# bioinfo-ut/GenomeTester4

Hardware: AMD Instinct MI355X
Metric: k-mers merged/sec, 2-list k=25 intersection (glistcompare -i), lists resident in HBM (higher is better)
Workload: dtype u64 keys + u32 counts

## Files before the change

### genometester4_amd/capi.py

```python
from __future__ import annotations

import ctypes as C
import os

import numpy as np

from .listio import RECORD_DTYPE

PKG_DIR = os.path.dirname(os.path.abspath(__file__))
LIB_PATH = os.environ.get("GT4HIP_LIB") or os.path.join(PKG_DIR, "libgt4hip.so")

OK = 0
EINVAL, ENODEVICE, ENOMEM, ERULE, EHIP, EWORDLEN, EINTERNAL = 1, 2, 3, 4, 5, 6, 7
EFORMAT = 11
MAKER_FORWARD_ONLY, MAKER_TEXT_ON_DEVICE = 1, 2
MAKER_ERR_START, MAKER_ERR_PLUS, MAKER_ERR_AT, MAKER_ERR_PLUS_EOF = 1, 2, 3, 4
OP_UNION, OP_INTRSEC, OP_DIFF1, OP_DIFF2 = 1, 2, 4, 8
RULE_DEFAULT, RULE_ADD, RULE_SUBTRACT, RULE_MIN, RULE_MAX, RULE_FIRST, RULE_SECOND, RULE_NUMBER = range(8)


class CompareParams(C.Structure):
    _fields_ = [("ops", C.c_uint32), ("rule", C.c_int32), ("cutoff", C.c_uint32), ("subtract", C.c_int32),
                ("count_override", C.c_uint32), ("count_only", C.c_int32)]

# ... 61 lines not shown


class MultiResult(C.Structure):
    _fields_ = [("n_words", C.c_uint64), ("total_count", C.c_uint64), ("out", C.c_void_p), ("device_ms", C.c_double),
                ("records_read", C.c_uint64), ("records_written", C.c_uint64)]


class CountTable(C.Structure):
    _fields_ = [("n_keys", C.c_uint64), ("n_lists", C.c_uint32), ("device_keys", C.c_void_p),
                ("device_counts", C.c_void_p), ("owner", C.c_void_p * 2), ("ragged", C.c_void_p)]


SYMBOLS = [
    "gt4hip_create", "gt4hip_destroy", "gt4hip_last_error", "gt4hip_strerror", "gt4hip_device_count",
    "gt4hip_device_info", "gt4hip_list_upload", "gt4hip_list_upload_index", "gt4hip_list_wrap", "gt4hip_list_alloc", "gt4hip_list_slice",
    "gt4hip_list_download", "gt4hip_list_download_range", "gt4hip_list_free", "gt4hip_list_n_words",
    "gt4hip_list_word_length", "gt4hip_list_device_ptr", "gt4hip_list_set_n_words", "gt4hip_list_sum_counts",
    "gt4hip_list_is_sorted", "gt4hip_list_lower_bound", "gt4hip_list_get_word", "gt4hip_compare",
    "gt4hip_union_multi", "gt4hip_intersect_multi", "gt4hip_union_table", "gt4hip_probe_table", "gt4hip_probe_table_ex", "gt4hip_table_compact", "gt4hip_table_download",
    "gt4hip_table_free", "gt4hip_generate", "gt4hip_generate_ex", "gt4hip_synchronize", "gt4hip_set_option",
    "gt4hip_get_counter", "gt4hip_device_memory", "gt4hip_list_upload_fd", "gt4hip_list_load_fd", "gt4hip_list_load",
    "gt4hip_list_write_fd", "gt4hip_lists_write_fd", "gt4hip_shard_first_key", "gt4hip_shard_cuts", "gt4hip_comm_unique_id", "gt4hip_comm_create", "gt4hip_comm_destroy", "gt4hip_comm_allgather_totals", "gt4hip_comm_allgather_u64", "gt4hip_context_device", "gt4hip_trim",
    "gt4hip_comm_rank", "gt4hip_comm_size", "gt4hip_comm_last_error", "gt4hip_comm_gatherv", "gt4hip_sort_words", "gt4hip_words_to_list",
    "gt4hip_device_words_to_list", "gt4hip_compare_mismatch", "gt4hip_mismatch_stats_get",
    "gt4hip_query_index_create", "gt4hip_query_index_free", "gt4hip_query_index_last_ms", "gt4hip_query_variants",
    "gt4hip_query_variant_mask", "gt4hip_query_lookup", "gt4hip_query_lookup_all", "gt4hip_list_count_stats",
    "gt4hip_list_count_split", "gt4hip_list_count_histogram", "gt4hip_list_gc",
    "gt4hip_location_index_create", "gt4hip_location_index_free", "gt4hip_location_index_list", "gt4hip_location_index_n_locations",
    "gt4hip_query_lookup_locations", "gt4hip_query_index_gather_ms",
    "gt4hip_text_to_words", "gt4hip_words_free", "gt4hip_words_download", "gt4hip_text_to_list",
    "gt4hip_sort_pairs", "gt4hip_pairs_to_index", "gt4hip_index_free",
    "gt4hip_list_subset", "gt4hip_subset_state_at",
    "gt4hip_text_to_locations", "gt4hip_locations_free", "gt4hip_pack_locations", "gt4hip_pairs_reserve", "gt4hip_pairs_release",
]

_lib = None


class Gt4HipError(RuntimeError):
    def __init__(self, code, msg):
        super().__init__("gt4hip error %d: %s" % (code, msg))
        self.code = code


def lib():
    global _lib
    if _lib is None:
        if not os.path.exists(LIB_PATH):
            raise ImportError("%s is missing: build it with `make -C genometester4_amd/csrc` "
                              "(there is no CPU fallback)" % LIB_PATH)
        L = C.CDLL(LIB_PATH)
        vp, u64, u32, i32 = C.c_void_p, C.c_uint64, C.c_uint32, C.c_int32
        sig = {
            "gt4hip_create": (C.c_int, [C.c_int, C.POINTER(vp)]),
            "gt4hip_destroy": (None, [vp]),
            "gt4hip_last_error": (C.c_char_p, [vp]),
            "gt4hip_strerror": (C.c_char_p, [C.c_int]),
            "gt4hip_device_count": (C.c_int, []),
            "gt4hip_device_info": (C.c_char_p, [vp]),
            "gt4hip_list_upload": (C.c_int, [vp, vp, u64, u32, C.POINTER(vp)]),
            "gt4hip_list_upload_index": (C.c_int, [vp, vp, u64, u64, u32, C.POINTER(vp)]),
            "gt4hip_list_wrap": (C.c_int, [vp, vp, u64, u32, C.POINTER(vp)]),
            "gt4hip_list_alloc": (C.c_int, [vp, u64, u32, C.POINTER(vp)]),
            "gt4hip_list_slice": (C.c_int, [vp, vp, u64, u64, C.POINTER(vp)]),
            "gt4hip_list_download": (C.c_int, [vp, vp, vp]),
            "gt4hip_list_download_range": (C.c_int, [vp, vp, u64, u64, vp]),
# ... 45 lines not shown
            "gt4hip_query_index_create": (C.c_int, [vp, vp, C.POINTER(vp)]),
            "gt4hip_query_index_free": (None, [vp]),
            "gt4hip_query_index_last_ms": (C.c_double, [vp]),
            "gt4hip_query_variants": (C.c_int, [u32, C.POINTER(QueryParams), C.POINTER(u64)]),
            "gt4hip_query_variant_mask": (C.c_int, [u32, C.POINTER(QueryParams), u64, C.POINTER(u64)]),
            "gt4hip_query_lookup": (C.c_int, [vp, vp, vp, u64, C.POINTER(QueryParams), vp, vp]),
            "gt4hip_query_lookup_all": (C.c_int, [vp, vp, vp, u64, C.POINTER(QueryParams), vp, u64, C.POINTER(u64)]),
            "gt4hip_location_index_create": (C.c_int, [vp, vp, u64, vp, u64, u32, u32, u32, u32, C.POINTER(vp)]),
            "gt4hip_location_index_free": (None, [vp]),
            "gt4hip_location_index_list": (vp, [vp]),
            "gt4hip_location_index_n_locations": (u64, [vp]),
            "gt4hip_query_lookup_locations": (C.c_int, [vp, vp, vp, vp, u64, C.POINTER(QueryParams), vp, u64, C.POINTER(u64), vp, u64, C.POINTER(u64)]),
            "gt4hip_query_index_gather_ms": (C.c_double, [vp]),
            "gt4hip_list_count_stats": (C.c_int, [vp, vp, C.POINTER(u32), C.POINTER(u32)]),
            "gt4hip_list_count_split": (C.c_int, [vp, vp, u32, C.POINTER(u64), C.POINTER(u64)]),
            "gt4hip_list_count_histogram": (C.c_int, [vp, vp, u32, vp]),
            "gt4hip_list_gc": (C.c_int, [vp, vp, C.POINTER(u64)]),
            "gt4hip_text_to_words": (C.c_int, [vp, vp, C.c_size_t, C.c_uint, C.c_uint, C.POINTER(MakerCarry), C.POINTER(MakerCarry),
                                               C.POINTER(vp), C.POINTER(u64), C.POINTER(u64)]),
            "gt4hip_words_free": (None, [vp, vp]),
            "gt4hip_words_download": (C.c_int, [vp, vp, u64, vp]),
            "gt4hip_text_to_list": (C.c_int, [vp, vp, C.c_size_t, C.c_uint, C.c_uint, C.POINTER(vp)]),
            "gt4hip_sort_pairs": (C.c_int, [vp, vp, vp, u64, u32]),
            "gt4hip_pairs_to_index": (C.c_int, [vp, vp, vp, u64, u32, u32, u32, C.POINTER(IndexArrays)]),
            "gt4hip_index_free": (None, [vp]),
            "gt4hip_text_to_locations": (C.c_int, [vp, vp, C.c_size_t, C.c_uint, C.c_uint, C.POINTER(LocationsCarry), C.POINTER(LocationsCarry),
                                                   vp, vp, u64, C.POINTER(LocationsPiece), C.POINTER(u64)]),
            "gt4hip_locations_free": (None, [vp]),
            "gt4hip_pack_locations": (C.c_int, [vp, vp, u64, u64, C.c_uint, C.c_uint]),
            "gt4hip_pairs_reserve": (C.c_int, [vp, u64, C.POINTER(vp), C.POINTER(vp)]),
            "gt4hip_pairs_release": (None, [vp]),
            "gt4hip_list_subset": (C.c_int, [vp, vp, C.POINTER(SubsetParams), C.POINTER(vp), C.POINTER(u64), C.POINTER(u64)]),
            "gt4hip_subset_state_at": (u64, [u64, u64]),
        }
        for name, (res, args) in sig.items():
            f = getattr(L, name)
            f.restype = res
            f.argtypes = args
        _lib = L
    return _lib


def comm_unique_id() -> bytes:
    buf = C.create_string_buffer(128)
    rc = lib().gt4hip_comm_unique_id(buf)
    if rc:
        raise Gt4HipError(rc, lib().gt4hip_comm_last_error().decode())
    return buf.raw


def comm_destroy(comm):
    lib().gt4hip_comm_destroy(comm)


class DeviceList:

    def __init__(self, ctx, handle):
        self.ctx = ctx
        self.h = handle
        ctx._lists.add(self)

    @property
    def n_words(self):
        return lib().gt4hip_list_n_words(self.h)

    @property
# ... 196 lines not shown
class Context:
    def __init__(self, device=0):
        import weakref
        self._lists = weakref.WeakSet()
        self.h = C.c_void_p()
        rc = lib().gt4hip_create(device, C.byref(self.h))
        if rc:
            raise Gt4HipError(rc, lib().gt4hip_last_error(None).decode())

    def _chk(self, rc):
        if rc:
            raise Gt4HipError(rc, lib().gt4hip_last_error(self.h).decode())

    def close(self):
        if self.h:
            for l in list(self._lists):
                l.free()
            lib().gt4hip_destroy(self.h)
            self.h = None

    def device_info(self):
        return lib().gt4hip_device_info(self.h).decode()

    def set_option(self, name, value):
        self._chk(lib().gt4hip_set_option(self.h, name.encode(), value))

    def get_counter(self, name) -> int:
        v = C.c_uint64()
        self._chk(lib().gt4hip_get_counter(self.h, name.encode(), C.byref(v)))
        return v.value

    def synchronize(self):
        self._chk(lib().gt4hip_synchronize(self.h))

    def shard_cuts(self, lists, n_shards):
        arr = (C.c_void_p * len(lists))(*[l.h for l in lists])
        out = (C.c_uint64 * n_shards)()
        self._chk(lib().gt4hip_shard_cuts(self.h, arr, len(lists), n_shards, out))
        return [int(x) for x in out]

    def words_to_list(self, words, word_length) -> "DeviceList":
        w = np.ascontiguousarray(words, dtype=np.uint64)
        h = C.c_void_p()
        self._chk(lib().gt4hip_words_to_list(self.h, w.ctypes.data if len(w) else None, len(w), word_length, C.byref(h)))
        return DeviceList(self, h)

    def text_to_words(self, text, word_length, flags=0, carry=None, n_bytes=None):
        out, d, n, at = MakerCarry(), C.c_void_p(), C.c_uint64(), C.c_uint64()
        if flags & MAKER_TEXT_ON_DEVICE:
            buf = C.c_void_p(text)
        else:
            buf, n_bytes = (C.c_char * max(len(text), 1)).from_buffer_copy(bytes(text) or b"\0"), len(text)
        rc = lib().gt4hip_text_to_words(self.h, buf, n_bytes, word_length, flags, C.byref(carry) if carry is not None else None,
                                        C.byref(out), C.byref(d), C.byref(n), C.byref(at))
        if rc:
            e = Gt4HipError(rc, lib().gt4hip_last_error(self.h).decode())
            e.error_offset, e.kind = at.value, out.error
            raise e
        words = np.empty(n.value, dtype=np.uint64)
        if n.value:
            rc = lib().gt4hip_words_download(self.h, d, n.value, words.ctypes.data)
            lib().gt4hip_words_free(self.h, d)
            self._chk(rc)
        return words, out

    def text_to_locations(self, pieces, word_length):
# ... 229 lines not shown
```

### genometester4_amd/csrc/gt4hip_api.hip

```cpp
#include "gt4hip_host.h"

#include <stdarg.h>
#include <stdio.h>
#include <stdlib.h>
#include <string.h>
#include <new>

using namespace gt4;

static thread_local char g_create_err[512] = "";

static void pool_flush (gt4hip_context *ctx);

int gt4hip_fail (gt4hip_context *ctx, int code, const char *fmt, ...)
{
  va_list ap;
  va_start (ap, fmt);
  vsnprintf (ctx ? ctx->err : g_create_err, 512, fmt, ap);
  va_end (ap);
  return code;
}

extern "C" const char *gt4hip_strerror (int code)
{
// ... 112 lines not shown
  HIPCHK (ctx, hipSetDevice (ctx->device));
  HIPCHK (ctx, hipStreamSynchronize (ctx->stream));
  pool_flush (ctx);
  return GT4HIP_OK;
}

extern "C" int gt4hip_device_memory (gt4hip_context *ctx, uint64_t *free_bytes, uint64_t *total_bytes)
{
  if (!ctx) return GT4HIP_EINVAL;
  HIPCHK (ctx, hipSetDevice (ctx->device));
  size_t f = 0, t = 0;
  HIPCHK (ctx, hipMemGetInfo (&f, &t));
  if (free_bytes) *free_bytes = (uint64_t) f + ctx->pool_bytes;
  if (total_bytes) *total_bytes = (uint64_t) t;
  return GT4HIP_OK;
}

extern "C" int gt4hip_set_option (gt4hip_context *ctx, const char *name, int64_t value)
{
  if (!ctx || !name) return GT4HIP_EINVAL;
  if (!strcmp (name, "two_pass")) ctx->two_pass = value != 0;
  else if (!strcmp (name, "pool")) {
    ctx->pool_enabled = value != 0 && ctx->pool;
    if (!ctx->pool_enabled) pool_flush (ctx);
  }
  else if (!strcmp (name, "pool_cap_mb")) {
    ctx->pool_cap = value > 0 ? (size_t) value << 20 : 0;
    if (ctx->pool_bytes > ctx->pool_cap) pool_flush (ctx);
  }
  else if (!strcmp (name, "grid")) ctx->grid_override = value;
  else if (!strcmp (name, "scan_group")) ctx->scan_group = (int) value;
  else if (!strcmp (name, "dynamic")) ctx->dynamic = (int) value;
  else if (!strcmp (name, "a_rows")) ctx->a_rows = (int) value;
  else if (!strcmp (name, "kway")) ctx->kway_enabled = (int) value;
  else if (!strcmp (name, "kway_max")) ctx->kway_max = value == 8 ? 8 : (value == 33 ? 33 : 32);
  else if (!strcmp (name, "kway_g")) ctx->kway_g = value;
  else if (!strcmp (name, "kway_vt")) ctx->kway_vt = value;
  else if (!strcmp (name, "spin_limit")) ctx->spin_limit = value > 0 ? (uint32_t) value : 0u;
  else if (!strcmp (name, "geom1")) ctx->force_geom = value != 0 ? 1 : 0;
  else if (!strcmp (name, "geom0")) ctx->force_geom = value != 0 ? -1 : 0;
  else return gt4hip_fail (ctx, GT4HIP_EINVAL, "unknown option %s", name);
  return GT4HIP_OK;
}

extern "C" int gt4hip_get_counter (gt4hip_context *ctx, const char *name, uint64_t *value)
{
  if (!ctx || !name || !value) return GT4HIP_EINVAL;
  if (!strcmp (name, "single_pass_fallbacks")) *value = ctx->single_pass_fallbacks;
  else if (!strcmp (name, "kway_calls")) *value = ctx->kway_calls;
  else if (!strcmp (name, "kway_overflows")) *value = ctx->kway_overflows;
  else if (!strcmp (name, "kway_declined")) *value = ctx->kway_declined;
  else if (!strcmp (name, "kway_splits")) *value = ctx->kway_splits;
  else if (!strcmp (name, "kway_shared_x100")) *value = ctx->kway_shared_x100;
  else if (!strcmp (name, "kway_width")) *value = ctx->kway_width;
  else if (!strcmp (name, "nway_kernel_us")) *value = (uint64_t) (ctx->nway_kernel_ms * 1000.0);
  else if (!strcmp (name, "nway_tiles")) *value = ctx->nway_tiles;
  else if (!strcmp (name, "nway_one_pass")) *value = (uint64_t) ctx->last_multi_one_pass;
  else if (!strcmp (name, "sort_us")) *value = (uint64_t) (ctx->sort_ms * 1000.0);
  else if (!strcmp (name, "fold_us")) *value = (uint64_t) (ctx->fold_ms * 1000.0);
  else if (!strcmp (name, "extract_us")) *value = (uint64_t) (ctx->extract_ms * 1000.0);
  else if (!strcmp (name, "maker_text_tile") || !strcmp (name, "maker_code_tile")) *value = GT4HIP_MAKER_TILE;
  else if (!strcmp (name, "table_us")) *value = (uint64_t) (ctx->table_ms * 1000.0);
  else if (!strcmp (name, "query_wide")) *value = ctx->query_wide;
  else if (!strcmp (name, "mm_wide_levels")) *value = ctx->mm_wide_levels;
  else if (!strcmp (name, "mm_unskipped_levels")) *value = ctx->mm_unskipped_levels;
  else if (!strcmp (name, "subset_passes")) *value = ctx->subset_passes;
  else if (!strcmp (name, "subset_tile")) *value = GT4HIP_SUBSET_TILE;
  else if (!strcmp (name, "subset_us")) *value = (uint64_t) (ctx->subset_ms * 1000.0);
  else return gt4hip_fail (ctx, GT4HIP_EINVAL, "unknown counter %s", name);
  return GT4HIP_OK;
}

extern "C" int gt4hip_synchronize (gt4hip_context *ctx)
{
  if (!ctx) return GT4HIP_EINVAL;
  HIPCHK (ctx, hipStreamSynchronize (ctx->stream));
  return GT4HIP_OK;
}


static void pool_flush (gt4hip_context *ctx)
// ... 298 lines not shown
```

### genometester4_amd/csrc/gt4hip_host.h

```cpp
#ifndef GT4HIP_HOST_H
#define GT4HIP_HOST_H

#include "../../include/gt4hip.h"
#include "gt4hip_internal.h"

#include <stddef.h>
#include <algorithm>
#include <utility>
#include <vector>

struct gt4hip_io;

struct gt4hip_context {
  int device;
  hipStream_t stream;
  hipEvent_t ev[4];
  int n_cus;
  int two_pass;
  int64_t grid_override;
  uint32_t spin_limit;
  int a_rows;
  int dynamic;
  int scan_group;
  int force_geom;
  uint64_t single_pass_fallbacks;
  std::vector<std::pair<void *, size_t>> *pool;
  int pool_enabled;
  size_t pool_bytes;
  size_t pool_cap;
  uint64_t *part;
  size_t part_bytes;
  unsigned long long *desc;
  size_t desc_bytes;
  unsigned long long *block_sums;
  size_t block_sums_bytes;
  gt4::PairControl *ctl;
  gt4::PairControl *ctl_host;
  unsigned long long *scratch;
  unsigned long long *scratch_host;
  uint64_t *kway_part;
  size_t kway_part_bytes;
  void *kway_cnt;
  size_t kway_cnt_bytes;
  uint64_t *kway_part2;
  size_t kway_part2_bytes;
  void *kway_need;
  size_t kway_need_bytes;
  uint64_t kway_splits;
  int kway_enabled;
  int kway_max;
  uint64_t kway_width;
  uint64_t kway_shared_x100;
  int64_t kway_g;
  int64_t kway_vt;
// ... 107 lines not shown
```

### genometester4_amd/csrc/gt4hip_internal.h

```cpp
#ifndef GT4HIP_INTERNAL_H
#define GT4HIP_INTERNAL_H

#include <hip/hip_runtime.h>
#include <stdint.h>

#include "gt4hip_pair_variant.h"

#ifdef GT4_PROFILE_PHASES
#define PROF(...) __VA_ARGS__
#else
#define PROF(...)
#endif

namespace gt4 {

struct PairOutputs {
  uint32_t *rec[4];
};

struct PairControl {
  unsigned long long n_words[4];
  unsigned long long total_count[4];
  unsigned int ticket;
  unsigned int error;
  unsigned int role;
  unsigned int pad;
  unsigned long long phase_cycles[24];
  unsigned long long resolve_stats[8];
};

hipError_t launch_partition (hipStream_t s, const uint32_t *A, uint64_t nA, const uint32_t *B, uint64_t nB,
                             uint64_t num_tiles, uint64_t tile_records, uint64_t *part);
hipError_t launch_pair_merge (hipStream_t s, const PairVariant &v, int grid, const uint32_t *A, uint64_t nA,
                              const uint32_t *B, uint64_t nB, const uint64_t *part, uint64_t num_tiles,
                              const PairParams &p, const PairOutputs &o, unsigned long long *desc,
                              PairControl *ctl);
hipError_t launch_scan_tiles (hipStream_t s, unsigned long long *desc, uint64_t num_tiles,
                              unsigned long long *block_sums);
hipError_t launch_generate (hipStream_t s, uint32_t *rec, uint64_t n, uint64_t stride, uint64_t seed,
                            uint64_t count_seed, uint32_t max_count, uint64_t mult, uint64_t add);
hipError_t launch_sum_counts (hipStream_t s, const uint32_t *rec, uint64_t n, unsigned long long *sum);
hipError_t launch_check_sorted (hipStream_t s, const uint32_t *rec, uint64_t n, unsigned int *bad);
hipError_t launch_lower_bound (hipStream_t s, const uint32_t *rec, uint64_t n, uint64_t key,
                               unsigned long long *idx);
hipError_t launch_extract_column (hipStream_t s, const uint32_t *rec, uint64_t n, uint32_t *counts, uint32_t n_lists, uint32_t column);
hipError_t launch_extract_keys (hipStream_t s, const uint32_t *rec, uint64_t n, unsigned long long *keys);
hipError_t launch_decode_index (hipStream_t s, const unsigned long long *kmers, uint64_t n, uint64_t num_locations, uint32_t *rec);

int merge_blocks_per_cu (const PairVariant &v);

}

#endif
```

### genometester4_amd/csrc/gt4hip_kernels.hip

```cpp
#define GT4_RESOLVE_LOOKBACK 3
#include "gt4hip_device.h"

#include <type_traits>

namespace gt4 {

namespace {


enum : u32 { KIND_SKIP = 0, KIND_A = 1, KIND_B = 2, KIND_BOTH = 3 };

struct StreamCoef {
  u32 m_f1, m_f2, m_min, m_max, m_sub2;
  u32 konst;
  u32 minz;
  u32 check_in;
  u32 lo;
  u32 cutoff;
  u32 subtract;
};

template <int S>
__device__ __forceinline__ StreamCoef make_coef (const PairParams &p)
{
  StreamCoef c;
  const u32 rule = p.rule[S];
  const u32 all = 0xffffffffu;
  c.m_f1 = (rule == 1 || rule == 5) ? all : 0u;
  c.m_f2 = (rule == 1 || rule == 6) ? all : 0u;
  c.m_min = (rule == 3 || rule == RULE_MINZ) ? all : 0u;
  c.m_max = (rule == 4 || rule == 2) ? all : 0u;
  c.m_sub2 = (rule == 2) ? all : 0u;
  c.konst = (rule == 7) ? p.count_override : 0u;
  c.minz = (rule == RULE_MINZ) ? 1u : 0u;
// ... 21 lines not shown
    in_ok = f1 >= c.cutoff && f2 < c.cutoff;
  }
  const u32 mx = f1 > f2 ? f1 : f2;
  u32 mn = f1 < f2 ? f1 : f2;
  if (c.minz && f1 == 0) mn = f2;
  u32 f = (c.m_f1 & f1) + (c.m_f2 & f2) + (c.m_min & mn) + (c.m_max & mx) - (c.m_sub2 & f2) + c.konst;
  bool keep = domain && (in_ok || !c.check_in) && f >= c.lo;
  if (S == 2) {
    const bool keep_sub = domain && f1 == f2 && f1 >= c.cutoff;
    keep = c.subtract ? keep_sub : keep;
    f = c.subtract ? f1 : f;
  }
  freq = f;
  return keep;
}

template <int S>
__device__ __forceinline__ bool eval_default (u32 kind, u32 fa, u32 fb, u32 cutoff, u32 &freq)
{
  if (S == 0) {
    freq = fa + fb;
    return kind != KIND_SKIP && (fa >= cutoff || fb >= cutoff) && freq != 0u;
  }
  if (S == 1) {
    freq = fa < fb ? fa : fb;
    return kind == KIND_BOTH && freq >= cutoff && freq != 0u;
  }
  const u32 f1 = S == 3 ? fb : fa, f2 = S == 3 ? fa : fb;
  freq = f1 - f2;
  return (kind & (S == 2 ? KIND_A : KIND_B)) != 0 && f1 >= cutoff && f2 < cutoff && freq != 0u;
}


__device__ __forceinline__ u64 merge_path (const u32 *__restrict__ A, u64 nA, const u32 *__restrict__ B, u64 nB, u64 diag, u64 lo, u64 hi)
{
  const u64 lo0 = diag > nB ? diag - nB : 0, hi0 = diag < nA ? diag : nA;
  if (lo < lo0) lo = lo0;
  if (hi > hi0) hi = hi0;
  while (lo < hi) {
    const u64 mid = (lo + hi) >> 1;
    if (load_key (A, mid) <= load_key (B, diag - 1 - mid)) lo = mid + 1;
    else hi = mid;
  }
  return lo;
}

constexpr u64 PART_COARSE = 64;

__global__ void k_partition_coarse (const u32 *__restrict__ A, u64 nA, const u32 *__restrict__ B, u64 nB, u64 num_tiles, u64 tile_records, u64 *__restrict__ coarse)
{
  const u64 c = (u64) blockIdx.x * blockDim.x + threadIdx.x;
  const u64 n_coarse = (num_tiles + PART_COARSE - 1) / PART_COARSE;
  if (c > n_coarse) return;
  const u64 total = nA + nB;
  u64 diag = c * PART_COARSE * tile_records;
  if (diag > total) diag = total;
  coarse[c] = merge_path (A, nA, B, nB, diag, 0, nA);
}

__global__ void k_partition (const u32 *__restrict__ A, u64 nA, const u32 *__restrict__ B, u64 nB,
                             u64 num_tiles, u64 tile_records, const u64 *__restrict__ coarse, u64 *__restrict__ part)
{
  const u64 t = (u64) blockIdx.x * blockDim.x + threadIdx.x;
  if (t > num_tiles) return;
  const u64 total = nA + nB;
  u64 diag = t * tile_records;
  if (diag > total) diag = total;
  const u64 c = t / PART_COARSE;
  u64 a = (t % PART_COARSE) ? merge_path (A, nA, B, nB, diag, coarse[c], coarse[c + 1]) : coarse[c], b = diag - a;
  if (a > 0 && b < nB && load_key (A, a - 1) == load_key (B, b)) b += 1;
  part[2 * t] = a;
  part[2 * t + 1] = b;
}


enum : int { STAGE_NONE = 0, STAGE_UNION = 1, STAGE_INTRSEC = 2, STAGE_ANY = 3, STAGE_UNION_LATE = 4, STAGE_COMPLEMENT = 5 };

template <int NT, int IPT, int OPS>
struct RankShared {
  static constexpr int CAP = NT * IPT;
  static constexpr int NCH = CAP / WAVE;
  static constexpr int STAGE_DW = OPS == STAGE_INTRSEC ? ((3 * (CAP / 2 + 1) + 3) & ~3)
                                  : ((OPS == STAGE_UNION || OPS == STAGE_COMPLEMENT) ? 3 * CAP
                                     : (OPS == STAGE_ANY ? 3 * (2 * CAP + 16) : (OPS == STAGE_UNION_LATE ? 3 * (CAP + 16) : 4)));
  static constexpr int STAGE_SLOTS = (OPS == STAGE_INTRSEC && IPT <= 4 && NT > 512) ? 4 : ((OPS == STAGE_ANY || OPS == STAGE_UNION_LATE) ? 1 : 2);
  alignas (16) u32 raw[3 * CAP];
  u32 stage[STAGE_SLOTS][STAGE_DW];
  u64 kmask[4][NCH + 1];
  u32 cpre[4][NCH + 1];
  u64 excl[4];
  u32 tot[4];
  u32 tick[3];
  u64 rng[3][4];
  u32 tile_id[3];
  u64 trash[WAVE];
};

__device__ __forceinline__ void store_lane0 (u64 *dst, u64 *trash, u64 v, int lane)
{
  u64 *const w = lane == 0 ? dst : trash + lane;
  *w = v;
}

// ... 815 lines not shown
  for (u64 i = (u64) blockIdx.x * blockDim.x + threadIdx.x; i < n; i += step) counts[i * n_lists + column] = rec[3 * i + 2];
}

__global__ void k_extract_keys (const u32 *__restrict__ rec, u64 n, u64 *__restrict__ keys)
{
  const u64 step = (u64) gridDim.x * blockDim.x;
  for (u64 i = (u64) blockIdx.x * blockDim.x + threadIdx.x; i < n; i += step) keys[i] = load_key (rec, i);
}

__global__ void k_decode_index (const u64 *__restrict__ kmers, u64 n, u64 num_locations, u32 *__restrict__ rec)
{
  const u64 step = (u64) gridDim.x * blockDim.x;
  for (u64 i = (u64) blockIdx.x * blockDim.x + threadIdx.x; i < n; i += step) {
    const u64 word = kmers[2 * i], loc = kmers[2 * i + 1];
    const u64 next = i + 1 < n ? kmers[2 * i + 3] : num_locations;
    rec[3 * i] = (u32) word;
    rec[3 * i + 1] = (u32) (word >> 32);
    rec[3 * i + 2] = (u32) (next - loc);
  }
}

inline int grid_for (u64 n, int block, int cap)
{
  u64 g = (n + block - 1) / block;
  if (g < 1) g = 1;
  if (g > (u64) cap) g = cap;
  return (int) g;
}

}


hipError_t launch_partition (hipStream_t s, const uint32_t *A, uint64_t nA, const uint32_t *B, uint64_t nB,
                             uint64_t num_tiles, uint64_t tile_records, uint64_t *part)
{
  u64 *const coarse = (u64 *) part + 2 * (num_tiles + 1);
  const u64 n_coarse = (num_tiles + PART_COARSE - 1) / PART_COARSE + 1;
  hipLaunchKernelGGL (k_partition_coarse, dim3 ((unsigned) ((n_coarse + 255) / 256)), dim3 (256), 0, s, A, nA, B, nB, num_tiles, tile_records, coarse);
  const u64 threads = num_tiles + 1;
  hipLaunchKernelGGL (k_partition, dim3 ((unsigned) ((threads + 255) / 256)), dim3 (256), 0, s, A, nA, B, nB, num_tiles, tile_records,
                      (const u64 *) coarse, (u64 *) part);
  return hipGetLastError ();
}

typedef void (*PairKernel) (const u32 *, u64, const u32 *, u64, u64 *, u64, PairParams, PairOutputs, u64 *, PairControl *);

template <int... Vs, class F>
static PairKernel lift (int v, F f)
{
  PairKernel k = nullptr;
  ((v == Vs ? (void) (k = f (std::integral_constant<int, Vs>{})) : (void) 0), ...);
  return k;
}

static PairKernel pair_kernel (const PairVariant &v)
{
  return lift<512, 1024> (v.nt, [&] (auto nt) {
    return lift<MODE_COUNT, MODE_LOOKBACK, MODE_OFFSETS> (v.mode, [&] (auto mode) {
      return lift<0, 1, 2, 4> (v.cls, [&] (auto cls) {
        return lift<0, 1, 2, 3> (v.fast, [&] (auto fast) {
          return lift<0, 3, 5, 15> (v.opset, [&] (auto opset) -> PairKernel {
            constexpr int NT = decltype (nt)::value, MODE = decltype (mode)::value, OPS = decltype (cls)::value, FAST = decltype (fast)::value,
                          OPSET = decltype (opset)::value, IPT = merge_ipt (NT, OPS);
            if constexpr (pair_variant_exists ({ NT, IPT, MODE, OPS, FAST, OPSET }))
              if (v.ipt == IPT) return k_pair_merge<NT, IPT, MODE, OPS, FAST, OPSET>;
            return nullptr;
          });
        });
      });
    });
  });
}

int merge_blocks_per_cu (const PairVariant &v)
// ... 82 lines not shown
```

### genometester4_amd/csrc/gt4hip_pair.hip

```cpp
#include "gt4hip_host.h"

#include <stdio.h>
#include <string.h>

using namespace gt4;

size_t gt4hip_lookback_desc_bytes (uint64_t tiles)
{
  const uint64_t rows = (tiles + 63) / 64;
  return (((size_t) rows * 64 * 16 + (size_t) (rows + 1) * 32 + (size_t) rows * 32) + 255) & ~(size_t) 255;
}

static size_t desc_bytes_for (uint64_t tiles)
{
  const size_t two = ((size_t) tiles * 32 + 255) & ~(size_t) 255;
  return std::max (gt4hip_lookback_desc_bytes (tiles), two);
}

int gt4hip_run_pair (gt4hip_context *ctx, const uint32_t *A, uint64_t nA, const uint32_t *B, uint64_t nB, const PairParams &p_in,
                     bool count_only, uint32_t *const dst[4], PairRun *run, bool force_two_pass)
{
  if (p_in.ops == 8u) {
    PairParams q = p_in;
    q.ops = 4u;
    q.rule[2] = p_in.rule[3];
    q.subtract = 0;
    uint32_t *const d2[4] = { NULL, NULL, dst ? dst[3] : NULL, NULL };
    const int rc = gt4hip_run_pair (ctx, B, nB, A, nA, q, count_only, d2, run, force_two_pass);
    run->n_words[3] = run->n_words[2];
    run->total_count[3] = run->total_count[2];
    run->n_words[2] = run->total_count[2] = 0;
    return rc;
  }
  if (p_in.ops == 2u && nA > nB && p_in.rule[1] != 2u && p_in.rule[1] != RULE_MINZ) {
    PairParams q = p_in;
    if (q.rule[1] == 5u) q.rule[1] = 6u;
    else if (q.rule[1] == 6u) q.rule[1] = 5u;
    return gt4hip_run_pair (ctx, B, nB, A, nA, q, count_only, dst, run, force_two_pass);
  }
  PairParams p = p_in;
  p.spin_limit = ctx->spin_limit;
  p.a_rows_off = ctx->a_rows < 0 ? 1u : 0u;
  memset (run, 0, sizeof *run);
  const uint64_t total = nA + nB;
  if (!total || !p.ops) return GT4HIP_OK;
  const bool two_pass = (ctx->two_pass || force_two_pass) && !count_only;
  const int geom = ctx->force_geom ? (ctx->force_geom > 0 ? 1 : 0) : (count_only ? 0 : 1);
  const PairVariant v1 = pair_variant (geom, (count_only || two_pass) ? MODE_COUNT : MODE_LOOKBACK, p);
  const PairVariant v2 = pair_variant (geom, MODE_OFFSETS, p);
  const uint64_t tile_records = merge_tile_records (v1);
  const uint64_t tiles = (total + tile_records - 1) / tile_records;
  if (tiles >= 0xffffffffull) return gt4hip_fail (ctx, GT4HIP_EINVAL, "lists too long: %llu merge tiles", (unsigned long long) tiles);
  run->tiles = tiles;
  p.dynamic = ctx->dynamic > 0 ? 1u : (ctx->dynamic < 0 ? 0u : ((geom == 1 && !count_only && p.ops != 4u && p.ops != 8u) ? 1u : 0u));
  p.scan_group = ctx->scan_group > 0 ? 1u : (ctx->scan_group < 0 ? 0u : (tiles > (20000ull << 6) ? 1u : 0u));
  int rc;
  if ((rc = gt4hip_grow (ctx, (void **) &ctx->part, &ctx->part_bytes, (size_t) (tiles + 1) * 16 + (size_t) (tiles / 64 + 3) * 8))) return rc;
  const bool need_desc = !count_only;
  if (need_desc && (rc = gt4hip_grow (ctx, (void **) &ctx->desc, &ctx->desc_bytes, desc_bytes_for (tiles)))) return rc;
  if (two_pass) {
    const size_t nb = (size_t) ((tiles + 2047) / 2048) * 32;
    if ((rc = gt4hip_grow (ctx, (void **) &ctx->block_sums, &ctx->block_sums_bytes, nb))) return rc;
  }
  int grid = ctx->n_cus * merge_blocks_per_cu (v1);
  if (ctx->grid_override > 0) grid = (int) ctx->grid_override;
  if ((uint64_t) grid > tiles + 1) grid = (int) tiles + 1;
  int grid2 = ctx->n_cus * merge_blocks_per_cu (v2);
  if ((uint64_t) grid2 > tiles) grid2 = (int) tiles;

  PairOutputs outs;
  for (int s = 0; s < 4; s++) outs.rec[s] = (count_only || !dst) ? NULL : dst[s];

  hipStream_t st = ctx->stream;
  HIPCHK (ctx, hipEventRecord (ctx->ev[0], st));
  HIPCHK (ctx, hipMemsetAsync (ctx->ctl, 0, sizeof (PairControl), st));
  if (need_desc && !two_pass) HIPCHK (ctx, hipMemsetAsync (ctx->desc, 0, desc_bytes_for (tiles), st));
  HIPCHK (ctx, launch_partition (st, A, nA, B, nB, tiles, tile_records, ctx->part));
  HIPCHK (ctx, hipEventRecord (ctx->ev[1], st));
  if (count_only) {
    HIPCHK (ctx, launch_pair_merge (st, v1, grid, A, nA, B, nB, ctx->part, tiles, p, outs, NULL, ctx->ctl));
  } else if (two_pass) {
    HIPCHK (ctx, launch_pair_merge (st, v1, grid, A, nA, B, nB, ctx->part, tiles, p, outs, ctx->desc, ctx->ctl));
    HIPCHK (ctx, launch_scan_tiles (st, ctx->desc, tiles, ctx->block_sums));
    HIPCHK (ctx, hipMemsetAsync (ctx->ctl, 0, sizeof (PairControl), st));
    HIPCHK (ctx, launch_pair_merge (st, v2, grid2, A, nA, B, nB, ctx->part, tiles, p, outs, ctx->desc, ctx->ctl));
  } else {
    HIPCHK (ctx, launch_pair_merge (st, v1, grid, A, nA, B, nB, ctx->part, tiles, p, outs, ctx->desc, ctx->ctl));
  }
  HIPCHK (ctx, hipEventRecord (ctx->ev[2], st));
  HIPCHK (ctx, hipMemcpyAsync (ctx->ctl_host, ctx->ctl, sizeof (PairControl), hipMemcpyDeviceToHost, st));
  HIPCHK (ctx, hipEventRecord (ctx->ev[3], st));
  HIPCHK (ctx, hipStreamSynchronize (st));
  float ms = 0;
  if (hipEventElapsedTime (&ms, ctx->ev[1], ctx->ev[2]) == hipSuccess) run->merge_ms = ms;
  if (hipEventElapsedTime (&ms, ctx->ev[0], ctx->ev[3]) == hipSuccess) run->device_ms = ms;
PROF (
  {
    static const char *names[8] = { "p0 wait+lds", "B0", "ring+fetch issue", "p1 rank", "B1", "p2 scan/publish", "B2+out+B3+scatter", "housekeeping" };
    unsigned long long tot = 0;
    for (int i = 0; i < 8; i++) tot += ctx->ctl_host->phase_cycles[i];
    fprintf (stderr, "[phases] tiles %llu merge %.3f ms:", (unsigned long long) tiles, run->merge_ms);
    for (int i = 0; i < 8; i++) fprintf (stderr, " %s %.1f%%", names[i], tot ? 100.0 * ctx->ctl_host->phase_cycles[i] / tot : 0.0);
    fprintf (stderr, " | avg cycles/tile %.0f\n", tiles ? (double) tot / tiles : 0.0);
    const unsigned long long *rs = ctx->ctl_host->resolve_stats;
    if (rs[0]) fprintf (stderr, "[resolve] sampled %llu avg spins %.2f first-look agg-not-ready %.1f%% carry-not-ready %.1f%% | [scanner] rows %llu polling rounds %llu rows complete at batch load %llu\n", rs[0], (double) rs[1] / rs[0], 100.0 * rs[3] / rs[0], 100.0 * rs[4] / rs[0], rs[7], rs[5], rs[6]);
  }
)
  if (ctx->ctl_host->error) {
    const unsigned flags = ctx->ctl_host->error;
    if (!two_pass && !count_only && !(flags & 2u)) {
      ctx->single_pass_fallbacks++;
      return gt4hip_run_pair (ctx, A, nA, B, nB, p, count_only, dst, run, true);
    }
    return gt4hip_fail (ctx, GT4HIP_EINTERNAL, "merge kernel reported error flags 0x%x", flags);
  }
  for (int s = 0; s < 4; s++) {
    run->n_words[s] = ctx->ctl_host->n_words[s];
    run->total_count[s] = ctx->ctl_host->total_count[s];
  }
  return GT4HIP_OK;
}

static uint64_t worst_case (int s, uint64_t nA, uint64_t nB)
{
  switch (s) {
    case 0: return nA + nB;
    case 1: return nA < nB ? nA : nB;
    case 2: return nA;
    default: return nB;
  }
}

int gt4hip_pair_with_outputs (gt4hip_context *ctx, const gt4hip_list *a, const gt4hip_list *b, const PairParams &p, bool count_only,
                              gt4hip_list *out[4], PairRun *run)
{
  TempLists made;
  gt4hip_list *use[4] = { NULL, NULL, NULL, NULL };
  uint32_t *dst[4] = { NULL, NULL, NULL, NULL };
  int rc;
  for (int s = 0; s < 4 && !count_only; s++) {
    if (!((p.ops >> s) & 1u)) continue;
    if ((rc = gt4hip_output_list (ctx, s, out[s], worst_case (s, a->n_words, b->n_words), a->word_length, made, &use[s]))) return rc;
    dst[s] = (uint32_t *) use[s]->dev;
  }
  if ((rc = gt4hip_run_pair (ctx, (const uint32_t *) a->dev, a->n_words, (const uint32_t *) b->dev, b->n_words, p, count_only, dst, run))) return rc;
  made.release ();
  for (int s = 0; s < 4; s++)
    if (use[s]) {
      out[s] = use[s];
      out[s]->n_words = run->n_words[s];
      out[s]->word_length = a->word_length;
    }
  return GT4HIP_OK;
// ... 38 lines not shown
```

### include/gt4hip.h

```cpp
#ifndef GT4HIP_H
#define GT4HIP_H

#include <stddef.h>
#include <stdint.h>

#ifdef __cplusplus
extern "C" {
#endif

#define GT4HIP_RECORD_BYTES 12u

enum {
  GT4HIP_OK = 0,
  GT4HIP_EINVAL = 1,
  GT4HIP_ENODEVICE = 2,
  GT4HIP_ENOMEM = 3,
  GT4HIP_ERULE = 4,
  GT4HIP_EHIP = 5,
  GT4HIP_EWORDLEN = 6,
  GT4HIP_EINTERNAL = 7,
  GT4HIP_ECALLBACK = 8,
  GT4HIP_EIO = 9,
  GT4HIP_ECOMM = 10,
  GT4HIP_EFORMAT = 11
// ... 299 lines not shown
  uint64_t max_position;
  uint64_t name_pos;
  uint64_t seq_pos;
  uint32_t seq_open;
  uint32_t pad;
} gt4hip_locations_carry;

typedef struct {
  uint64_t n_words;
  uint64_t n_subseqs;
  const gt4hip_subseq *subseqs;
  uint64_t closed_seq_len;
  uint32_t closed, pad;
} gt4hip_locations_piece;

int gt4hip_text_to_locations (gt4hip_context *ctx, const void *text, size_t n_bytes, unsigned word_length, unsigned flags,
                              const gt4hip_locations_carry *in, gt4hip_locations_carry *out, uint64_t *d_words,
                              uint64_t *d_raw, uint64_t capacity, gt4hip_locations_piece *piece, uint64_t *error_offset);
void gt4hip_locations_free (gt4hip_context *ctx);
int gt4hip_pack_locations (gt4hip_context *ctx, uint64_t *d_raw, uint64_t n, uint64_t file, unsigned subseq_bits,
                           unsigned pos_bits);
int gt4hip_pairs_reserve (gt4hip_context *ctx, uint64_t n_pairs, uint64_t **d_words, uint64_t **d_values);
void gt4hip_pairs_release (gt4hip_context *ctx);


int gt4hip_generate (gt4hip_context *ctx, gt4hip_list *list, uint64_t n, uint64_t seed, uint32_t max_count);
int gt4hip_generate_ex (gt4hip_context *ctx, gt4hip_list *list, uint64_t n, uint64_t key_seed, uint64_t count_seed,
                        uint32_t max_count, uint64_t mult, uint64_t add);

int gt4hip_synchronize (gt4hip_context *ctx);

int gt4hip_set_option (gt4hip_context *ctx, const char *name, int64_t value);
int gt4hip_get_counter (gt4hip_context *ctx, const char *name, uint64_t *value);

#ifdef __cplusplus
}
#endif
#endif
```

Measured before the change: 366.0 billion.

## Use interpolation-guided co-rank search and fold control zeroing into partition kernel

Replaces the plain binary merge-path search with a guided search that first interpolates the split point from key slopes over the coarse boundaries, then falls back to bisection. It also removes the two hipMemsetAsync calls for the control block and lookback descriptors, which the partition kernel now zeroes with a grid-stride loop. Together these aim to cut partition latency and per-call launch overhead before the merge. The cost is floating-point heuristics in the search and more complex zeroing address logic. A host-side partition query API and a partition timing counter are also added.

```diff
diff --git a/genometester4_amd/capi.py b/genometester4_amd/capi.py
--- a/genometester4_amd/capi.py
+++ b/genometester4_amd/capi.py
@@ -117,6 +117,7 @@
     "gt4hip_sort_pairs", "gt4hip_pairs_to_index", "gt4hip_index_free",
     "gt4hip_list_subset", "gt4hip_subset_state_at",
     "gt4hip_text_to_locations", "gt4hip_locations_free", "gt4hip_pack_locations", "gt4hip_pairs_reserve", "gt4hip_pairs_release",
+    "gt4hip_pair_partition",
 ]
 
 _lib = None
@@ -228,6 +229,7 @@
             "gt4hip_pairs_release": (None, [vp]),
             "gt4hip_list_subset": (C.c_int, [vp, vp, C.POINTER(SubsetParams), C.POINTER(vp), C.POINTER(u64), C.POINTER(u64)]),
             "gt4hip_subset_state_at": (u64, [u64, u64]),
+            "gt4hip_pair_partition": (C.c_int, [vp, vp, vp, u64, vp]),
         }
         for name, (res, args) in sig.items():
             f = getattr(L, name)
@@ -490,6 +492,12 @@
 
     def synchronize(self):
         self._chk(lib().gt4hip_synchronize(self.h))
+
+    def pair_partition(self, a: "DeviceList", b: "DeviceList", tile_records):
+        tiles = (a.n_words + b.n_words + tile_records - 1) // tile_records
+        part = np.empty((tiles + 1, 2), dtype=np.uint64)
+        self._chk(lib().gt4hip_pair_partition(self.h, a.h, b.h, tile_records, part.ctypes.data))
+        return part
 
     def shard_cuts(self, lists, n_shards):
         arr = (C.c_void_p * len(lists))(*[l.h for l in lists])
diff --git a/genometester4_amd/csrc/gt4hip_api.hip b/genometester4_amd/csrc/gt4hip_api.hip
--- a/genometester4_amd/csrc/gt4hip_api.hip
+++ b/genometester4_amd/csrc/gt4hip_api.hip
@@ -168,6 +168,7 @@
   else if (!strcmp (name, "scan_group")) ctx->scan_group = (int) value;
   else if (!strcmp (name, "dynamic")) ctx->dynamic = (int) value;
   else if (!strcmp (name, "a_rows")) ctx->a_rows = (int) value;
+  else if (!strcmp (name, "part_guided")) ctx->part_guided = (int) value;
   else if (!strcmp (name, "kway")) ctx->kway_enabled = (int) value;
   else if (!strcmp (name, "kway_max")) ctx->kway_max = value == 8 ? 8 : (value == 33 ? 33 : 32);
   else if (!strcmp (name, "kway_g")) ctx->kway_g = value;
@@ -183,6 +184,7 @@
 {
   if (!ctx || !name || !value) return GT4HIP_EINVAL;
   if (!strcmp (name, "single_pass_fallbacks")) *value = ctx->single_pass_fallbacks;
+  else if (!strcmp (name, "partition_us")) *value = (uint64_t) (ctx->partition_ms * 1000.0);
   else if (!strcmp (name, "kway_calls")) *value = ctx->kway_calls;
   else if (!strcmp (name, "kway_overflows")) *value = ctx->kway_overflows;
   else if (!strcmp (name, "kway_declined")) *value = ctx->kway_declined;
diff --git a/genometester4_amd/csrc/gt4hip_corank.h b/genometester4_amd/csrc/gt4hip_corank.h
--- /dev/null
+++ b/genometester4_amd/csrc/gt4hip_corank.h
@@ -0,0 +1,132 @@
+#ifndef GT4HIP_CORANK_H
+#define GT4HIP_CORANK_H
+
+#include <stdint.h>
+
+#if defined(__HIPCC__)
+#define GT4_HD __host__ __device__ __attribute__ ((always_inline))
+#else
+#define GT4_HD __attribute__ ((always_inline))
+#endif
+
+namespace gt4 {
+
+constexpr uint64_t PART_COARSE = 64;
+
+constexpr int CORANK_KEY_PROBES = 3;
+constexpr int CORANK_GUIDED_MAX = 1 + CORANK_KEY_PROBES;
+constexpr uint64_t CORANK_NARROW = 32;
+constexpr uint64_t CORANK_SHRINK = 4;
+constexpr double CORANK_STRETCH = 8.0;
+
+struct CorankGuide {
+  uint64_t d0, a0, d1, a1;
+};
+
+GT4_HD inline uint32_t corank_bisect_bound (uint64_t w)
+{
+  uint32_t n = 0;
+  while (w) {
+    n++;
+    w >>= 1;
+  }
+  return n;
+}
+
+template <class KeyA, class KeyB>
+GT4_HD inline uint64_t corank_search (KeyA key_a, uint64_t nA, KeyB key_b, uint64_t nB, uint64_t diag, uint64_t lo, uint64_t hi,
+                                      bool guided, const CorankGuide &guide, uint32_t *probes = nullptr)
+{
+  const uint64_t lo0 = diag > nB ? diag - nB : 0, hi0 = diag < nA ? diag : nA;
+  if (lo < lo0) lo = lo0;
+  if (hi > hi0) hi = hi0;
+  int phase = 2, left = 0;
+  uint64_t next = 0;
+  double slope = 0.0;
+  if (guided && lo < hi && hi - lo > CORANK_NARROW && guide.d1 > guide.d0 && guide.a1 >= guide.a0) {
+    const uint64_t dd = guide.d1 - guide.d0, da = guide.a1 - guide.a0, db = dd >= da ? dd - da : 0;
+    const uint64_t off = diag > guide.d0 ? (diag < guide.d1 ? diag - guide.d0 : dd) : 0;
+    const double r = (double) da * ((double) off / (double) dd);
+    next = guide.a0 + (r < (double) da ? (uint64_t) r : da);
+    phase = 0;
+    const uint64_t b0 = guide.d0 - guide.a0;
+    bool stretches = true;
+    if (da > 1 && guide.a1 <= nA) {
+      const uint64_t k0 = key_a (guide.a0), k1 = key_a (guide.a1 - 1);
+      const double s = (double) (k1 - k0) / (double) (da - 1);
+      slope += s;
+      stretches = stretches && (double) (key_a (guide.a0 + 1) - k0) * CORANK_STRETCH < s && (double) (k1 - key_a (guide.a1 - 2)) * CORANK_STRETCH < s;
+    }
+    if (db > 1 && b0 + db <= nB) {
+      const uint64_t k0 = key_b (b0), k1 = key_b (b0 + db - 1);
+      const double s = (double) (k1 - k0) / (double) (db - 1);
+      slope += s;
+      stretches = stretches && (double) (key_b (b0 + 1) - k0) * CORANK_STRETCH < s && (double) (k1 - key_b (b0 + db - 2)) * CORANK_STRETCH < s;
+    }
+    left = slope > 0.0 ? CORANK_KEY_PROBES : 0;
+    if (slope > 0.0 && stretches) phase = 2;
+  }
+  uint32_t n = 0;
+  while (lo < hi) {
+    uint64_t mid = lo + ((hi - lo) >> 1);
+    if (phase < 2) mid = next < lo ? lo : (next >= hi ? hi - 1 : next);
+    const uint64_t ka = key_a (mid), kb = key_b (diag - 1 - mid);
+    n++;
+    const uint64_t w0 = hi - lo;
+    const bool up = ka <= kb;
+    if (up) lo = mid + 1;
+    else hi = mid;
+    if (phase == 2) continue;
+    const uint64_t w = hi - lo;
+    if ((phase == 1 && w > w0 / CORANK_SHRINK) || left == 0 || w <= CORANK_NARROW) {
+      phase = 2;
+      continue;
+    }
+    left--;
+    phase = 1;
+    double step = (double) (up ? kb - ka : ka - kb) / slope;
+    step += 3.0 * __builtin_sqrt (step) + 2.0;
+    const uint64_t su = step < (double) (w - 1) ? (uint64_t) step : w - 1;
+    next = up ? lo + su : hi - 1 - su;
+  }
+  if (probes) *probes = n;
+  return lo;
+}
+
+template <class KeyA, class KeyB>
+GT4_HD inline void corank_tile_boundary (KeyA key_a, uint64_t nA, KeyB key_b, uint64_t nB, uint64_t tile_records, uint64_t t, uint64_t c_lo,
+                                         uint64_t c_hi, bool guided, uint64_t *a_out, uint64_t *b_out, uint32_t *probes = nullptr)
+{
+  const uint64_t total = nA + nB, span = PART_COARSE * tile_records, c = t / PART_COARSE;
+  uint64_t diag = t * tile_records;
+  if (diag > total) diag = total;
+  uint64_t a = c_lo;
+  if (probes) *probes = 0;
+  if (t % PART_COARSE) {
+    CorankGuide g;
+    g.d0 = c * span < total ? c * span : total;
+    g.d1 = (c + 1) * span < total ? (c + 1) * span : total;
+    g.a0 = c_lo;
+    g.a1 = c_hi;
+    a = corank_search (key_a, nA, key_b, nB, diag, c_lo, c_hi, guided, g, probes);
+  }
+  uint64_t b = diag - a;
+  if (a > 0 && b < nB && key_a (a - 1) == key_b (b)) b += 1;
+  *a_out = a;
+  *b_out = b;
+}
+
+template <class KeyA, class KeyB>
+GT4_HD inline uint64_t corank_coarse_boundary (KeyA key_a, uint64_t nA, KeyB key_b, uint64_t nB, uint64_t tile_records, uint64_t c, bool guided,
+                                               uint32_t *probes = nullptr)
+{
+  const uint64_t total = nA + nB;
+  uint64_t diag = c * PART_COARSE * tile_records;
+  if (diag > total) diag = total;
+  const CorankGuide g = { 0, 0, total, nA };
+  return corank_search (key_a, nA, key_b, nB, diag, 0, nA, guided, g, probes);
+}
+
+}
+
+#endif
diff --git a/genometester4_amd/csrc/gt4hip_host.h b/genometester4_amd/csrc/gt4hip_host.h
--- a/genometester4_amd/csrc/gt4hip_host.h
+++ b/genometester4_amd/csrc/gt4hip_host.h
@@ -20,6 +20,8 @@
   int64_t grid_override;
   uint32_t spin_limit;
   int a_rows;
+  int part_guided;
+  double partition_ms;
   int dynamic;
   int scan_group;
   int force_geom;
diff --git a/genometester4_amd/csrc/gt4hip_internal.h b/genometester4_amd/csrc/gt4hip_internal.h
--- a/genometester4_amd/csrc/gt4hip_internal.h
+++ b/genometester4_amd/csrc/gt4hip_internal.h
@@ -29,8 +29,15 @@
   unsigned long long resolve_stats[8];
 };
 
+struct PartZero {
+  void *ctl;
+  uint32_t ctl_chunks, ops;
+  unsigned long long *desc;
+  uint64_t rows;
+};
+
 hipError_t launch_partition (hipStream_t s, const uint32_t *A, uint64_t nA, const uint32_t *B, uint64_t nB,
-                             uint64_t num_tiles, uint64_t tile_records, uint64_t *part);
+                             uint64_t num_tiles, uint64_t tile_records, uint64_t *part, bool guided, const PartZero &zero);
 hipError_t launch_pair_merge (hipStream_t s, const PairVariant &v, int grid, const uint32_t *A, uint64_t nA,
                               const uint32_t *B, uint64_t nB, const uint64_t *part, uint64_t num_tiles,
                               const PairParams &p, const PairOutputs &o, unsigned long long *desc,
diff --git a/genometester4_amd/csrc/gt4hip_kernels.hip b/genometester4_amd/csrc/gt4hip_kernels.hip
--- a/genometester4_amd/csrc/gt4hip_kernels.hip
+++ b/genometester4_amd/csrc/gt4hip_kernels.hip
@@ -1,5 +1,6 @@
 #define GT4_RESOLVE_LOOKBACK 3
 #include "gt4hip_device.h"
+#include "gt4hip_corank.h"
 
 #include <type_traits>
 
@@ -87,43 +88,56 @@
 }
 
 
-__device__ __forceinline__ u64 merge_path (const u32 *__restrict__ A, u64 nA, const u32 *__restrict__ B, u64 nB, u64 diag, u64 lo, u64 hi)
-{
-  const u64 lo0 = diag > nB ? diag - nB : 0, hi0 = diag < nA ? diag : nA;
-  if (lo < lo0) lo = lo0;
-  if (hi > hi0) hi = hi0;
-  while (lo < hi) {
-    const u64 mid = (lo + hi) >> 1;
-    if (load_key (A, mid) <= load_key (B, diag - 1 - mid)) lo = mid + 1;
-    else hi = mid;
-  }
-  return lo;
-}
-
-constexpr u64 PART_COARSE = 64;
-
-__global__ void k_partition_coarse (const u32 *__restrict__ A, u64 nA, const u32 *__restrict__ B, u64 nB, u64 num_tiles, u64 tile_records, u64 *__restrict__ coarse)
+struct KeyOf {
+  const u32 *rec;
+  __device__ __forceinline__ u64 operator() (u64 i) const { return load_key (rec, i); }
+};
+
+__global__ void k_partition_coarse (const u32 *__restrict__ A, u64 nA, const u32 *__restrict__ B, u64 nB, u64 num_tiles, u64 tile_records, u64 *__restrict__ coarse,
+                                    int guided)
 {
   const u64 c = (u64) blockIdx.x * blockDim.x + threadIdx.x;
   const u64 n_coarse = (num_tiles + PART_COARSE - 1) / PART_COARSE;
   if (c > n_coarse) return;
-  const u64 total = nA + nB;
-  u64 diag = c * PART_COARSE * tile_records;
-  if (diag > total) diag = total;
-  coarse[c] = merge_path (A, nA, B, nB, diag, 0, nA);
+  coarse[c] = corank_coarse_boundary (KeyOf{ A }, nA, KeyOf{ B }, nB, tile_records, c, guided != 0);
+}
+
+__device__ __forceinline__ u32x4 *zero_chunk (const PartZero &z, u64 j)
+{
+  if (j < z.ctl_chunks) return reinterpret_cast<u32x4 *> (z.ctl) + j;
+  j -= z.ctl_chunks;
+  u32x4 *const agg = reinterpret_cast<u32x4 *> (z.desc), *const carry = agg + z.rows * 64, *const rowsum = carry + 2 * (z.rows + 1);
+#pragma unroll
+  for (u32 s = 0; s < 4; s++) {
+    if (!((z.ops >> s) & 1u)) continue;
+    const u64 n_agg = z.rows * 16;
+    if (j < n_agg) return agg + s * n_agg + j;
+    j -= n_agg;
+    const u64 c0 = (s * (z.rows + 1)) >> 1, c1 = ((s + 1) * (z.rows + 1) + 1) >> 1;
+    if (j < c1 - c0) return carry + c0 + j;
+    j -= c1 - c0;
+    const u64 r0 = (s * z.rows) >> 1, r1 = ((s + 1) * z.rows + 1) >> 1;
+    if (j < r1 - r0) return rowsum + r0 + j;
+    j -= r1 - r0;
+  }
+  return nullptr;
 }
 
 __global__ void k_partition (const u32 *__restrict__ A, u64 nA, const u32 *__restrict__ B, u64 nB,
-                             u64 num_tiles, u64 tile_records, const u64 *__restrict__ coarse, u64 *__restrict__ part)
+                             u64 num_tiles, u64 tile_records, const u64 *__restrict__ coarse, u64 *__restrict__ part, int guided, PartZero z)
 {
   const u64 t = (u64) blockIdx.x * blockDim.x + threadIdx.x;
+  const u64 threads = (u64) gridDim.x * blockDim.x;
+  for (u64 i = t;; i += threads) {
+    u32x4 *const chunk = zero_chunk (z, i);
+    if (!chunk) break;
+    *chunk = u32x4{ 0u, 0u, 0u, 0u };
+  }
   if (t > num_tiles) return;
-  const u64 total = nA + nB;
-  u64 diag = t * tile_records;
-  if (diag > total) diag = total;
   const u64 c = t / PART_COARSE;
-  u64 a = (t % PART_COARSE) ? merge_path (A, nA, B, nB, diag, coarse[c], coarse[c + 1]) : coarse[c], b = diag - a;
-  if (a > 0 && b < nB && load_key (A, a - 1) == load_key (B, b)) b += 1;
+  uint64_t a, b;
+  const u64 c_lo = coarse[c], c_hi = (t % PART_COARSE) ? coarse[c + 1] : c_lo;
+  corank_tile_boundary (KeyOf{ A }, nA, KeyOf{ B }, nB, tile_records, t, c_lo, c_hi, guided != 0, &a, &b);
   part[2 * t] = a;
   part[2 * t + 1] = b;
 }
@@ -1005,14 +1019,15 @@
 
 
 hipError_t launch_partition (hipStream_t s, const uint32_t *A, uint64_t nA, const uint32_t *B, uint64_t nB,
-                             uint64_t num_tiles, uint64_t tile_records, uint64_t *part)
+                             uint64_t num_tiles, uint64_t tile_records, uint64_t *part, bool guided, const PartZero &zero)
 {
   u64 *const coarse = (u64 *) part + 2 * (num_tiles + 1);
   const u64 n_coarse = (num_tiles + PART_COARSE - 1) / PART_COARSE + 1;
-  hipLaunchKernelGGL (k_partition_coarse, dim3 ((unsigned) ((n_coarse + 255) / 256)), dim3 (256), 0, s, A, nA, B, nB, num_tiles, tile_records, coarse);
+  hipLaunchKernelGGL (k_partition_coarse, dim3 ((unsigned) ((n_coarse + 255) / 256)), dim3 (256), 0, s, A, nA, B, nB, num_tiles, tile_records, coarse,
+                      guided ? 1 : 0);
   const u64 threads = num_tiles + 1;
   hipLaunchKernelGGL (k_partition, dim3 ((unsigned) ((threads + 255) / 256)), dim3 (256), 0, s, A, nA, B, nB, num_tiles, tile_records,
-                      (const u64 *) coarse, (u64 *) part);
+                      (const u64 *) coarse, (u64 *) part, guided ? 1 : 0, zero);
   return hipGetLastError ();
 }
 
diff --git a/genometester4_amd/csrc/gt4hip_pair.hip b/genometester4_amd/csrc/gt4hip_pair.hip
--- a/genometester4_amd/csrc/gt4hip_pair.hip
+++ b/genometester4_amd/csrc/gt4hip_pair.hip
@@ -15,6 +15,21 @@
 {
   const size_t two = ((size_t) tiles * 32 + 255) & ~(size_t) 255;
   return std::max (gt4hip_lookback_desc_bytes (tiles), two);
+}
+
+static PartZero pair_zero (gt4hip_context *ctx, uint64_t tiles, uint32_t ops, bool desc)
+{
+  static_assert (sizeof (PairControl) % 16 == 0, "the control block is zeroed in 16-byte chunks");
+  PartZero z;
+  memset (&z, 0, sizeof z);
+  z.ctl = ctx->ctl;
+  z.ctl_chunks = (uint32_t) (sizeof (PairControl) / 16);
+  if (desc) {
+    z.ops = ops;
+    z.desc = ctx->desc;
+    z.rows = (tiles + 63) / 64;
+  }
+  return z;
 }
 
 int gt4hip_run_pair (gt4hip_context *ctx, const uint32_t *A, uint64_t nA, const uint32_t *B, uint64_t nB, const PairParams &p_in,
@@ -73,9 +88,7 @@
 
   hipStream_t st = ctx->stream;
   HIPCHK (ctx, hipEventRecord (ctx->ev[0], st));
-  HIPCHK (ctx, hipMemsetAsync (ctx->ctl, 0, sizeof (PairControl), st));
-  if (need_desc && !two_pass) HIPCHK (ctx, hipMemsetAsync (ctx->desc, 0, desc_bytes_for (tiles), st));
-  HIPCHK (ctx, launch_partition (st, A, nA, B, nB, tiles, tile_records, ctx->part));
+  HIPCHK (ctx, launch_partition (st, A, nA, B, nB, tiles, tile_records, ctx->part, ctx->part_guided >= 0, pair_zero (ctx, tiles, p.ops, need_desc && !two_pass)));
   HIPCHK (ctx, hipEventRecord (ctx->ev[1], st));
   if (count_only) {
     HIPCHK (ctx, launch_pair_merge (st, v1, grid, A, nA, B, nB, ctx->part, tiles, p, outs, NULL, ctx->ctl));
@@ -94,6 +107,7 @@
   float ms = 0;
   if (hipEventElapsedTime (&ms, ctx->ev[1], ctx->ev[2]) == hipSuccess) run->merge_ms = ms;
   if (hipEventElapsedTime (&ms, ctx->ev[0], ctx->ev[3]) == hipSuccess) run->device_ms = ms;
+  if (hipEventElapsedTime (&ms, ctx->ev[0], ctx->ev[1]) == hipSuccess) ctx->partition_ms = ms;
 PROF (
   {
     static const char *names[8] = { "p0 wait+lds", "B0", "ring+fetch issue", "p1 rank", "B1", "p2 scan/publish", "B2+out+B3+scatter", "housekeeping" };
@@ -119,6 +133,22 @@
     run->total_count[s] = ctx->ctl_host->total_count[s];
   }
   return GT4HIP_OK;
+}
+
+extern "C" int gt4hip_pair_partition (gt4hip_context *ctx, const gt4hip_list *a, const gt4hip_list *b, uint64_t tile_records, uint64_t *host_part)
+{
+  if (!ctx || !a || !b || !host_part || !tile_records) return GT4HIP_EINVAL;
+  if (a->word_length != b->word_length) return gt4hip_fail (ctx, GT4HIP_EWORDLEN, "word lengths differ (%u != %u)", b->word_length, a->word_length);
+  HIPCHK (ctx, hipSetDevice (ctx->device));
+  const uint64_t tiles = (a->n_words + b->n_words + tile_records - 1) / tile_records;
+  if (tiles >= 0xffffffffull) return gt4hip_fail (ctx, GT4HIP_EINVAL, "lists too long: %llu merge tiles", (unsigned long long) tiles);
+  int rc;
+  if ((rc = gt4hip_grow (ctx, (void **) &ctx->part, &ctx->part_bytes, (size_t) (tiles + 1) * 16 + (size_t) (tiles / 64 + 3) * 8))) return rc;
+  PartZero none;
+  memset (&none, 0, sizeof none);
+  HIPCHK (ctx, launch_partition (ctx->stream, (const uint32_t *) a->dev, a->n_words, (const uint32_t *) b->dev, b->n_words, tiles, tile_records, ctx->part,
+                                 ctx->part_guided >= 0, none));
+  return gt4hip_read_back (ctx, host_part, ctx->part, (size_t) (tiles + 1) * 16, "gt4hip_pair_partition: reading the tile ranges back failed");
 }
 
 static uint64_t worst_case (int s, uint64_t nA, uint64_t nB)
diff --git a/include/gt4hip.h b/include/gt4hip.h
--- a/include/gt4hip.h
+++ b/include/gt4hip.h
@@ -355,6 +355,7 @@
 
 int gt4hip_set_option (gt4hip_context *ctx, const char *name, int64_t value);
 int gt4hip_get_counter (gt4hip_context *ctx, const char *name, uint64_t *value);
+int gt4hip_pair_partition (gt4hip_context *ctx, const gt4hip_list *a, const gt4hip_list *b, uint64_t tile_records, uint64_t *host_part);
 
 #ifdef __cplusplus
 }
```

New measurement: 375.8 billion (median of 6 runs). 1.03x the previous value.
